# KumarRobotics/top_down_renderer

Hardware: AMD Instinct MI355X
Metric: particle-updates/sec (render+score+resample) (higher is better)
Workload: dtype f32

## Files before the change

top_down_renderer_amd/csrc/tdr_score_su.h:

```cpp
#ifndef TDR_SCORE_SU_H_
#define TDR_SCORE_SU_H_
#include "tdr_common.h"

static inline int64_t su_npad(int64_t n, int nb) { return cdiv(n + 63 * std::min<int64_t>(nb, n), 64) * 64; }
bool tdr_su_shape_ok(int nb, int nr, int group, int64_t n_total);
struct SuWs {
  int64_t tab_su, desc, bbox, keys_in, keys_out, vals_in, vals_out, ints, slots, sort_tmp, ray_tab, ray_desc, ray_multi, ray_rad, total;
  int64_t slots2, wave_tmp;
};
#define TDR_SU_TAIL_INTS 10
#define TDR_RAY_MAX_SPLIT 8
SuWs tdr_su_ws(int nb, int nr, int group, int64_t n);

struct SuLaunch {
  const tdr_map_desc* map;
  const float* tab;
  bool uniform_scale;
  const float* scan_pk;
  int nb, nr, rf;
  float res;
  const float* st;
  int64_t cap, n;
  const int32_t* perm;
  int group, nchunks;
  int64_t npad;
  float* part;
  int ray_split;
  const float* fac;
  float uscale;
  int32_t* ws;
  float span;
  float wave_span = 0.f;
};
int tdr_su_prepare(const SuLaunch& L, const SuWs& W, hipStream_t s, const int32_t** slots_out, const int32_t** counts_out);
int tdr_su_order(const SuLaunch& L, const SuWs& W, hipStream_t s, const int32_t** slots_out, const int32_t** counts_out);
struct SpanTuner {
  int64_t shape = -1;
  int phase = -2;
  int settled_launches = 0;
  int trial = 0;
  float best = 16.f;
  float round_best = 16.f, best_ms = 3.0e38f;
  hipEvent_t e0 = nullptr, e1 = nullptr;
  bool open = false, pending = false;
  int64_t trial_calls = 0;
};
float tdr_su_span_begin(SpanTuner* t, int64_t shape, hipStream_t s);
void tdr_su_span_end(SpanTuner* t, hipStream_t s);
float tdr_su_wave_span();
int tdr_su_score(const SuLaunch& L, const SuWs& W, hipStream_t s);
bool tdr_ray_map_ok(const tdr_map_desc* map);
int64_t tdr_ray_padded_samples(int nb, int nr);
int tdr_ray_splits(int nb, int nr, int64_t n, bool block_major = false);
bool tdr_ray_block_major(const SuLaunch& L);
int tdr_ray_prepare(const SuLaunch& L, const SuWs& W, hipStream_t s);
int tdr_ray_score(const SuLaunch& L, const SuWs& W, hipStream_t s);
#endif
```

top_down_renderer_amd/csrc/tdr_score_su.hip:

```cpp
#include <rocprim/device/device_radix_sort.hpp>

#include <atomic>

#include "tdr_score_dev.h"
#include "tdr_score_su.h"
#include "tdr_score_su_asm.h"

#define SU_CODE_FULL 0xFFu
#define SU_CODE_FULL_ALL 0xFEu
#define SU_CODE_PAD 0xFDu
#define SU_NSECT 8
#define SU_BOX_WORDS 4096

struct SuArgs {
  const uint32_t* crec;
  const uint32_t* kmask;
  int kcolw;
  unsigned kmask_off;
  const uint32_t* dict_int;
  int dict_n, ctiles_r;
  int pkcol;
  const int32_t* inexact;
  int rows, cols;
  float resolution;
  const float* tab_su;
  const uint32_t* desc;
  const float* bbox;
  const float* scan_pk;
  int nb, nr;
  float res;
  const float* st;
  int64_t cap;
  const int32_t* slots;
  const int32_t* nslots;
  int group, nchunks, ncls;
  int64_t npad;
  uint32_t* part;
  uint32_t* stats;
};

__global__ __launch_bounds__(256) void su_prep_kernel(const float* __restrict__ tab, const float* __restrict__ scan_pk,
                                                      int nb, int nr, int rf, int ncls, int ckconst, unsigned pbase,
                                                      unsigned plane_bytes, int group, int nchunks,
                                                      const float* __restrict__ dict, int dict_n, float* __restrict__ tab_su,
                                                      uint32_t* __restrict__ desc) {
  const int64_t t = (int64_t)blockIdx.x * blockDim.x + threadIdx.x;
  bool bad = false;
  for (int k = threadIdx.x; k < dict_n; k += blockDim.x) bad |= !(fabsf(dict[k]) <= 3.402823466e+38f);
  const bool dict_bad = __syncthreads_or(bad);
  const int64_t total = (int64_t)nchunks * nb * group;
  const bool live = t < total;
  const int64_t tt = live ? t : 0;
  const int jj = (int)(tt % group);
  const int64_t q = tt / group;
  const int i = (int)(q % nb), chunk = (int)(q / nb);
  const int j = chunk * group + jj;
  float tx = 0.f, ty = 0.f, val = 0.f;
  uint32_t code = SU_CODE_PAD, ckc = (uint32_t)ckconst, sh = 0;
  if (live && j >= nr) {
    const int64_t k = (int64_t)(nr - 1) * nb + i;
    tx = tab[2 * k];
    ty = tab[2 * k + 1];
  }
  if (live && j < nr) {
    code = 0;
    const int64_t k = (int64_t)j * nb + i;
    tx = tab[2 * k];
    ty = tab[2 * k + 1];
    const float* r = scan_pk + k * rf;
    int nz = 0, first = 0;
    bool finite = true;
    for (int c = 0; c < ncls; c++) {
      finite &= fabsf(r[c]) <= 3.402823466e+38f;
      if (r[c] != 0.f) {
        if (!nz) first = c;
        nz++;
      }
    }
    if (dict_bad || !finite) { code = SU_CODE_FULL_ALL; val = r[rf - 1]; }
    else if (nz == 1) { code = (uint32_t)first + 1u; val = r[first]; ckc = pbase + (uint32_t)first * plane_bytes; }
    else if (nz > 1) { code = SU_CODE_FULL; val = r[rf - 1]; }
  }
  uint32_t anyfull = code >= SU_CODE_FULL_ALL ? 1u : 0u;
  anyfull |= __shfl_xor(anyfull, 1);
  anyfull |= __shfl_xor(anyfull, 2);
  if (!live) return;
  tab_su[2 * t] = tx;
  tab_su[2 * t + 1] = ty;
  desc[4 * t] = code;
  desc[4 * t + 1] = (uint32_t)val;
  desc[4 * t + 2] = ckc;
  desc[4 * t + 3] = sh | (((jj & 3) == 0 && anyfull) ? 0x80000000u : 0u);
}

__global__ __launch_bounds__(256) void su_bbox_kernel(const float* __restrict__ tab_su, int nb, int nr, int group,
                                                      float* __restrict__ bbox) {
  const int chunk = blockIdx.x, sect = blockIdx.y;
  const int i0 = (int)((int64_t)sect * nb / SU_NSECT), i1 = (int)((int64_t)(sect + 1) * nb / SU_NSECT);
  const int gn = min(nr - chunk * group, group);
  float lo0 = 3.402823466e+38f, hi0 = -3.402823466e+38f, lo1 = lo0, hi1 = hi0;
  const int cnt = (i1 - i0) * gn;
  for (int t = threadIdx.x; t < cnt; t += 256) {
    const int i = i0 + t / gn, jj = t % gn;
    const float* e = tab_su + (((int64_t)chunk * nb + i) * group + jj) * 2;
    lo0 = fminf(lo0, e[0]); hi0 = fmaxf(hi0, e[0]);
    lo1 = fminf(lo1, e[1]); hi1 = fmaxf(hi1, e[1]);
  }
  __shared__ float red[4][256];
  red[0][threadIdx.x] = lo0; red[1][threadIdx.x] = hi0; red[2][threadIdx.x] = lo1; red[3][threadIdx.x] = hi1;
  __syncthreads();
  for (int d = 128; d > 0; d >>= 1) {
    if ((int)threadIdx.x < d) {
      red[0][threadIdx.x] = fminf(red[0][threadIdx.x], red[0][threadIdx.x + d]);
      red[1][threadIdx.x] = fmaxf(red[1][threadIdx.x], red[1][threadIdx.x + d]);
      red[2][threadIdx.x] = fminf(red[2][threadIdx.x], red[2][threadIdx.x + d]);
      red[3][threadIdx.x] = fmaxf(red[3][threadIdx.x], red[3][threadIdx.x + d]);
    }
    __syncthreads();
  }
  if (threadIdx.x < 4) bbox[((int64_t)chunk * SU_NSECT + sect) * 4 + threadIdx.x] = red[threadIdx.x][0];
}

__global__ __launch_bounds__(256) void su_key_kernel(const float* __restrict__ st, int64_t cap, int64_t n,
                                                     const int32_t* __restrict__ perm, int nb, float span,
                                                     uint32_t* __restrict__ keys, int32_t* __restrict__ vals,
                                                     int* __restrict__ cnt) {
  extern __shared__ int hist[];
  for (int k = threadIdx.x; k <= nb; k += 256) hist[k] = 0;
  __syncthreads();
  const int64_t t = (int64_t)blockIdx.x * blockDim.x + threadIdx.x;
  if (t < n) {
    const int32_t p = perm ? perm[t] : (int32_t)t;
    uint32_t key = (uint32_t)rot_shift_dev(st[TDR_ST_THETA * cap + p], nb);
    if (span > 0.f) {
      auto centre = [&](int64_t q, float& x, float& y) {
        const float sc = st[TDR_ST_SCALE * cap + q];
        x = st[TDR_ST_DX * cap + q] * sc + st[TDR_ST_INIT_X * cap + q];
        y = st[TDR_ST_DY * cap + q] * sc + st[TDR_ST_INIT_Y * cap + q];
      };
      const int64_t ta = t >= 32 ? t - 32 : 0, tb = t + 32 < n ? t + 32 : n - 1;
      float x0, y0, x1, y1;
      centre(perm ? perm[ta] : ta, x0, y0);
      centre(perm ? perm[tb] : tb, x1, y1);
      if (!(fabsf(x1 - x0) <= span && fabsf(y1 - y0) <= span)) key = (uint32_t)nb;
    }
    keys[t] = key;
    vals[t] = p;
    atomicAdd(&hist[key], 1);
  }
  __syncthreads();
  for (int k = threadIdx.x; k <= nb; k += 256)
    if (hist[k]) atomicAdd(&cnt[k], hist[k]);
}

__global__ __launch_bounds__(256) void su_offsets_kernel(const int* __restrict__ cnt, int nkeys, int* __restrict__ start,
                                                         int* __restrict__ slot_start, int* __restrict__ counts) {
  __shared__ int sa[256], sb[256];
  int carry_a = 0, carry_b = 0;
  for (int base = 0; base < nkeys; base += 256) {
    const int k = base + threadIdx.x;
    const int c = k < nkeys ? cnt[k] : 0;
    const int cp = k < nkeys - 1 ? (c + 63) & ~63 : c;
    sa[threadIdx.x] = c;
    sb[threadIdx.x] = cp;
    __syncthreads();
    for (int d = 1; d < 256; d <<= 1) {
      const int va = threadIdx.x >= d ? sa[threadIdx.x - d] : 0;
      const int vb = threadIdx.x >= d ? sb[threadIdx.x - d] : 0;
      __syncthreads();
      sa[threadIdx.x] += va;
      sb[threadIdx.x] += vb;
      __syncthreads();
    }
    if (k < nkeys) {
      start[k] = carry_a + sa[threadIdx.x] - c;
      slot_start[k] = carry_b + sb[threadIdx.x] - cp;
    }
    carry_a += sa[255];
    carry_b += sb[255];
    __syncthreads();
  }
  if (threadIdx.x == 0) {
    const int sparse = cnt[nkeys - 1];
    counts[0] = carry_b - sparse;
    counts[1] = sparse;
    counts[2] = carry_b;
  }
}

__global__ __launch_bounds__(256) void su_scatter_kernel(const uint32_t* __restrict__ keys, const int32_t* __restrict__ vals,
                                                         int64_t n, const int* __restrict__ start,
                                                         const int* __restrict__ slot_start, int32_t* __restrict__ slots) {
  const int64_t t = (int64_t)blockIdx.x * blockDim.x + threadIdx.x;
  if (t >= n) return;
  const uint32_t k = keys[t];
  slots[slot_start[k] + ((int)t - start[k])] = vals[t];
}

__global__ __launch_bounds__(256) void su_wave_far_kernel(const float* __restrict__ st, int64_t cap, const int32_t* __restrict__ slots,
                                                          const int32_t* __restrict__ counts, float wave_span,
                                                          int32_t* __restrict__ keep, int32_t* __restrict__ moved) {
  const int lane = threadIdx.x & 63;
  const int64_t w = (int64_t)blockIdx.x * 4 + (threadIdx.x >> 6), base = w * 64;
  if (base >= (int64_t)counts[0]) return;
  const int32_t p = slots[base + lane];
  float x0 = 3.0e38f, x1 = -3.0e38f, y0 = 3.0e38f, y1 = -3.0e38f;
  if (p >= 0) {
    const float sc = st[TDR_ST_SCALE * cap + p];
    const float x = st[TDR_ST_DX * cap + p] * sc + st[TDR_ST_INIT_X * cap + p];
    const float y = st[TDR_ST_DY * cap + p] * sc + st[TDR_ST_INIT_Y * cap + p];
    x0 = x1 = x;
    y0 = y1 = y;
  }
#pragma unroll
  for (int d = 32; d > 0; d >>= 1) {
    x0 = fminf(x0, __shfl_xor(x0, d)); x1 = fmaxf(x1, __shfl_xor(x1, d));
    y0 = fminf(y0, __shfl_xor(y0, d)); y1 = fmaxf(y1, __shfl_xor(y1, d));
  }
  const int nvalid = __popcll(__ballot(p >= 0));
  const bool far = (x1 - x0 > wave_span) || (y1 - y0 > wave_span);
  if (lane == 0) {
    keep[w] = far ? 0 : 1;
    moved[w] = far ? nvalid : 0;
  }
}
__global__ __launch_bounds__(256) void su_compact_offsets_kernel(int32_t* __restrict__ keep, int32_t* __restrict__ moved,
                                                                 int32_t* __restrict__ counts, int32_t* __restrict__ old_counts) {
  __shared__ int sa[256], sb[256];
  const int c0 = counts[0], c1 = counts[1], c2 = counts[2];
  const int nw = c0 >> 6;
  int carry_a = 0, carry_b = 0;
  for (int base = 0; base < nw; base += 256) {
    const int w = base + threadIdx.x;
    const int a = w < nw ? keep[w] : 0, b = w < nw ? moved[w] : 0;
    sa[threadIdx.x] = a;
    sb[threadIdx.x] = b;
    __syncthreads();
    for (int d = 1; d < 256; d <<= 1) {
      const int va = threadIdx.x >= d ? sa[threadIdx.x - d] : 0;
      const int vb = threadIdx.x >= d ? sb[threadIdx.x - d] : 0;
      __syncthreads();
      sa[threadIdx.x] += va;
      sb[threadIdx.x] += vb;
      __syncthreads();
    }
    if (w < nw) {
      keep[w] = a ? (carry_a + sa[threadIdx.x] - a) * 64 : -1;
      moved[w] = carry_b + sb[threadIdx.x] - b;
    }
    carry_a += sa[255];
    carry_b += sb[255];
    __syncthreads();
  }
  if (threadIdx.x == 0) {
    old_counts[0] = c0; old_counts[1] = c1; old_counts[2] = c2;
    counts[0] = carry_a * 64;
    counts[1] = c1 + carry_b;
    counts[2] = carry_a * 64 + c1 + carry_b;
  }
}
__global__ __launch_bounds__(256) void su_compact_scatter_kernel(const int32_t* __restrict__ slots, const int32_t* __restrict__ keep,
                                                                 const int32_t* __restrict__ moved,
                                                                 const int32_t* __restrict__ counts,
                                                                 const int32_t* __restrict__ old_counts, int32_t* __restrict__ out) {
  const int64_t t = (int64_t)blockIdx.x * blockDim.x + threadIdx.x;
  const int oc0 = old_counts[0], oc1 = old_counts[1];
  if (t >= (int64_t)oc0 + oc1) return;
  const int32_t p = slots[t];
  if (t >= oc0) {
    out[(int64_t)counts[0] + (t - oc0)] = p;
    return;
  }
  const int64_t w = t >> 6;
  const int32_t k = keep[w];
  const uint64_t valid = __ballot(p >= 0);
  if (k >= 0) {
    out[(int64_t)k + (t & 63)] = p;
  } else if (p >= 0) {
    const int rank = __popcll(valid & (((uint64_t)1 << (t & 63)) - 1));
    out[(int64_t)counts[0] + oc1 + moved[w] + rank] = p;
  }
}
__global__ void su_copy_slots_kernel(const int32_t* __restrict__ src, const int32_t* __restrict__ counts, int32_t* __restrict__ dst) {
  const int64_t t = (int64_t)blockIdx.x * blockDim.x + threadIdx.x;
  if (t < (int64_t)counts[2]) dst[t] = src[t];
}

struct SuLds {
  uint32_t dict[TDR_CMAP_MAX_DICT];
  uint32_t bits[SU_BOX_WORDS];
  int box[4];
};

template <int NV4, bool KSLOT, bool USCALE>
__global__ __launch_bounds__(256) __attribute__((amdgpu_waves_per_eu(6, 8))) void score_polar_su_kernel(SuArgs a) {
  constexpr int RF = 4 * NV4;
  constexpr int ND = CmapShape<RF, KSLOT>::ND, CW = CmapShape<RF, KSLOT>::CW;
  constexpr bool ASM_LOOP = CW == 2 && ND == 6;
  __shared__ SuLds lds;
  if (int_form_off(a.inexact)) return;
  for (int t = threadIdx.x; t < a.dict_n; t += 256) lds.dict[t] = a.dict_int[t];
  const int lane = threadIdx.x & 63, wave = __builtin_amdgcn_readfirstlane(threadIdx.x >> 6);
  const int64_t nsl = (int64_t)__builtin_amdgcn_readfirstlane(*a.nslots);
  if ((int64_t)blockIdx.x * 256 >= nsl) return;
  const int64_t base = ((int64_t)blockIdx.x * 4 + wave) * 64;
  const bool active = base < nsl;
  const int32_t sp = active ? a.slots[base + lane] : -1;
  const int32_t p0 = a.slots[active ? base : (int64_t)blockIdx.x * 256];
  const int64_t p = sp >= 0 ? sp : p0;
  const float scale = a.st[TDR_ST_SCALE * a.cap + p];
  const float cx = a.st[TDR_ST_DX * a.cap + p] * scale + a.st[TDR_ST_INIT_X * a.cap + p];
  const float cy = a.st[TDR_ST_DY * a.cap + p] * scale + a.st[TDR_ST_INIT_Y * a.cap + p];
  const float off0 = cy / a.resolution;
  const float off1 = cx / a.resolution;
  const int shift = __builtin_amdgcn_readfirstlane(rot_shift_dev(a.st[TDR_ST_THETA * a.cap + p], a.nb));
  const int nb = a.nb, G = a.group;
  const int j0 = blockIdx.y * G, gn = min(a.nr - j0, G);
  const float rmaxf = (float)a.rows, cmaxf = (float)a.cols;
  const int ckcol = a.ctiles_r * 128 - 16 * CW;
  const int pkcol = a.pkcol;
  const uint32_t ckconst = (uint32_t)(a.ctiles_r * 128 + 128);
  auto su_rec_const = [&](uint32_t cd) -> uint32_t {
    return cd != 0 && cd < SU_CODE_PAD ? ckconst + 4u * (((cd - 1u) * 11u) >> 5) : ckconst;
  };
  typedef const float __attribute__((address_space(4))) * tdr_const_f;
  typedef const uint32_t __attribute__((address_space(4))) * tdr_const_u;
  const tdr_const_f tbase = (tdr_const_f)a.tab_su + (int64_t)blockIdx.y * nb * G * 2;
  const tdr_const_u dbase = (tdr_const_u)a.desc + (int64_t)blockIdx.y * nb * G * 4;
  const tdr_const_f bbase = (tdr_const_f)a.bbox + (int64_t)blockIdx.y * SU_NSECT * 4;
  const tdr_const_f scanc = (tdr_const_f)a.scan_pk;
  const uint32_t* __restrict__ crec = a.crec;
  const uint32_t* __restrict__ kmask = a.kmask;
  const unsigned lds_base = (unsigned)(uintptr_t)&lds;
  const unsigned lbits_lds = (unsigned)(uintptr_t)&lds.bits[0];

  typedef float tdr_v2f __attribute__((ext_vector_type(2)));
  const tdr_v2f offv = {off0, off1};
  typedef const uint32_t __attribute__((address_space(3))) * tdr_lds_u;
  auto lds_word = [](unsigned byte_addr) -> uint32_t { return *reinterpret_cast<tdr_lds_u>((uintptr_t)byte_addr); };
  const char* __restrict__ crecb = reinterpret_cast<const char*>(a.crec);
  auto map_dword = [&](unsigned off) -> uint32_t { return *reinterpret_cast<const uint32_t*>(crecb + off); };
  auto map_ushort = [&](unsigned off) -> uint32_t { return *reinterpret_cast<const uint16_t*>(crecb + off); };
  const bool weird = !(fabsf(off0) <= 1e9f) || !(fabsf(off1) <= 1e9f) || (!USCALE && !(fabsf(scale * a.res) <= 1e9f));
  auto field = [&](const uint32_t (&w)[CW], int k) -> uint32_t {
    const uint32_t ww = w[k / 3];
    const int sh = 10 * (k % 3);
    const uint32_t boff = sh ? ((ww >> sh) & 0xFFCu) : (ww & 0xFFCu);
    return *reinterpret_cast<const uint32_t*>(reinterpret_cast<const char*>(lds.dict) + boff);
  };
  auto field1 = [&](uint32_t ww, int k) -> uint32_t {
    const int sh = 10 * (k % 3);
    const uint32_t boff = sh ? ((ww >> sh) & 0xFFCu) : (ww & 0xFFCu);
    return *reinterpret_cast<const uint32_t*>(reinterpret_cast<const char*>(lds.dict) + boff);
  };

  uint64_t acc[ND];
#pragma unroll
  for (int k = 0; k < ND; k++) acc[k] = 0;
  uint32_t norm = 0;
  uint32_t known = 0;

  auto single_class = [&](uint32_t cd, uint32_t v, uint32_t ww) {
    switch (cd) {
#define SU_CASE(K)                                                                                 \
  case K + 1:                                                                                      \
    if constexpr (K < ND) {                                                                        \
      const uint32_t m = field1(ww, K < ND ? K : 0);                                               \
      asm volatile("v_mad_u64_u32 %0, vcc, %1, %2, %0" : "+v"(acc[K < ND ? K : 0]) : "s"(v), "v"(m) : "vcc"); \
    }                                                                                              \
    break;
      SU_CASE(0) SU_CASE(1) SU_CASE(2) SU_CASE(3) SU_CASE(4) SU_CASE(5)
      SU_CASE(6) SU_CASE(7) SU_CASE(8) SU_CASE(9) SU_CASE(10)
#undef SU_CASE
      default: break;
    }
  };
  auto single_class_plane = [&](uint32_t cd, uint32_t v, uint32_t cell) {
    const uint32_t m = *reinterpret_cast<const uint32_t*>(reinterpret_cast<const char*>(lds.dict) + (cell & 0xFFCu));
    switch (cd) {
#define SU_CASE(K)                                                                                 \
  case K + 1:                                                                                      \
    if constexpr (K < ND) {                                                                        \
      asm volatile("v_mad_u64_u32 %0, vcc, %1, %2, %0" : "+v"(acc[K < ND ? K : 0]) : "s"(v), "v"(m) : "vcc"); \
    }                                                                                              \
    break;
      SU_CASE(0) SU_CASE(1) SU_CASE(2) SU_CASE(3) SU_CASE(4) SU_CASE(5)
      SU_CASE(6) SU_CASE(7) SU_CASE(8) SU_CASE(9) SU_CASE(10)
#undef SU_CASE
      default: break;
    }
  };
  auto full_bin = [&](uint32_t cd, uint32_t v, const uint32_t (&wr)[CW], int kbit, int64_t bin) {
    const tdr_const_f S = scanc + bin * RF;
    norm += v & (0u - (uint32_t)kbit);
#pragma unroll
    for (int k = 0; k < ND; k++) {
      const float sk = S[k];
      if (sk != 0.f) acc[k] += (uint64_t)(uint32_t)sk * (uint64_t)field(wr, k);
    }
  };
  auto cell = [&](float tx, float ty, int& ri, int& ci) {
    tdr_v2f pv = {tx, ty};
    if constexpr (!USCALE) pv = (pv * scale) * a.res;
    pv = pv + offv;
    tdr_v2f qv = {__builtin_amdgcn_fmed3f(pv.x, -1.f, rmaxf), __builtin_amdgcn_fmed3f(pv.y, -1.f, cmaxf)};
    qv = qv + 0.49999997f;
    asm("v_cvt_flr_i32_f32 %0, %1" : "=v"(ri) : "v"(qv.x));
    asm("v_cvt_flr_i32_f32 %0, %1" : "=v"(ci) : "v"(qv.y));
  };

  auto cpp_step = [&](int i, int r, int jj, int krow4, int kconst) {
    const tdr_const_f T = tbase + ((int64_t)i * G + jj) * 2;
    const tdr_const_u D = dbase + ((int64_t)r * G + jj) * 4;
    uint32_t val[4];
    uint32_t code[4], pad[4];
    uint32_t w[4], bits[4];
    int cis[4];
    unsigned offs[4];
#pragma unroll
    for (int u = 0; u < 4; u++) {
      code[u] = D[4 * u];
      pad[u] = code[u] == SU_CODE_PAD ? 0u : 0xFFFFFFFFu;
      code[u] = code[u] == SU_CODE_PAD ? 0u : code[u];
      val[u] = D[4 * u + 1];
      const uint32_t ckc = su_rec_const(code[u]);
      int ri, ci;
      cell(T[2 * u], T[2 * u + 1], ri, ci);
      cis[u] = ci;
      int wa;
      asm("v_mad_i32_i24 %0, %1, %2, %3" : "=v"(wa) : "v"(ri), "v"(krow4), "s"(kconst));
      const int cw5 = ci >> 5;
      unsigned la;
      asm("v_lshl_add_u32 %0, %1, 2, %2" : "=v"(la) : "v"(cw5), "v"(wa));
      bits[u] = lds_word(la);
      w[u] = 0;
      offs[u] = 0;
      if (code[u] != 0) {
        int t1, t2;
        const int cq = ci >> 2;
        asm("v_mad_i32_i24 %0, %1, %2, %3" : "=v"(t1) : "v"(cq), "v"(ckcol), "s"(ckc));
        asm("v_lshl_add_u32 %0, %1, %2, %3" : "=v"(t2) : "v"(ci), "n"(CW == 1 ? 2 : (CW == 2 ? 3 : 4)), "v"(t1));
        asm("v_lshl_add_u32 %0, %1, %2, %3" : "=v"(offs[u]) : "v"(ri), "n"(CW == 1 ? 4 : (CW == 2 ? 5 : 6)), "v"(t2));
        w[u] = map_dword(offs[u]);
      }
    }
#pragma unroll
    for (int u = 0; u < 4; u++) {
      const uint32_t cd = code[u];
      int kmsk;
      asm("v_bfe_i32 %0, %1, %2, 1" : "=v"(kmsk) : "v"(bits[u]), "v"(cis[u]));
      known -= (uint32_t)kmsk & pad[u];
      if (cd != 0) {
        if (cd < SU_CODE_FULL_ALL) {
          norm += (uint32_t)kmsk & val[u];
          single_class(cd, val[u], w[u]);
        } else {
          uint32_t wr[CW];
          wr[0] = w[u];
#pragma unroll
          for (int d = 1; d < CW; d++)
            wr[d] = map_dword(offs[u] + 4u * d);
          full_bin(cd, val[u], wr, kmsk & 1, (int64_t)(j0 + jj + u) * nb + r);
        }
      }
    }
  };
  auto cpp_step_plane = [&](int i, int r, int jj, int krow4, int kconst) {
    const tdr_const_f T = tbase + ((int64_t)i * G + jj) * 2;
    const tdr_const_u D = dbase + ((int64_t)r * G + jj) * 4;
    uint32_t val[4];
    uint32_t code[4], pad[4];
    uint32_t w[4], bits[4];
    int cis[4];
#pragma unroll
    for (int u = 0; u < 4; u++) {
      code[u] = D[4 * u];
      pad[u] = code[u] == SU_CODE_PAD ? 0u : 0xFFFFFFFFu;
      code[u] = code[u] == SU_CODE_PAD ? 0u : code[u];
      val[u] = D[4 * u + 1];
      const uint32_t pkc = D[4 * u + 2];
      int ri, ci;
      cell(T[2 * u], T[2 * u + 1], ri, ci);
      cis[u] = ci;
      int wa;
      asm("v_mad_i32_i24 %0, %1, %2, %3" : "=v"(wa) : "v"(ri), "v"(krow4), "s"(kconst));
      const int cw5 = ci >> 5;
      unsigned la;
      asm("v_lshl_add_u32 %0, %1, 2, %2" : "=v"(la) : "v"(cw5), "v"(wa));
      bits[u] = lds_word(la);
      w[u] = 0;
      if (code[u] != 0) {
        int t1, t2;
        unsigned off;
        const int cq = ci >> 3;
        asm("v_mad_i32_i24 %0, %1, %2, %3" : "=v"(t1) : "v"(cq), "v"(pkcol), "s"(pkc));
        asm("v_lshl_add_u32 %0, %1, 1, %2" : "=v"(t2) : "v"(ci), "v"(t1));
        asm("v_lshl_add_u32 %0, %1, 4, %2" : "=v"(off) : "v"(ri), "v"(t2));
        w[u] = map_ushort(off);
      }
// ... 36 lines not shown
          const uint32_t ckc = su_rec_const(D[4 * u]);
          int t1, t2;
          const int cq = ci >> 2;
          asm("v_mad_i32_i24 %0, %1, %2, %3" : "=v"(t1) : "v"(cq), "v"(ckcol), "s"(ckc));
          asm("v_lshl_add_u32 %0, %1, %2, %3" : "=v"(t2) : "v"(ci), "n"(CW == 1 ? 2 : (CW == 2 ? 3 : 4)), "v"(t1));
          asm("v_lshl_add_u32 %0, %1, %2, %3" : "=v"(off) : "v"(ri), "n"(CW == 1 ? 4 : (CW == 2 ? 5 : 6)), "v"(t2));
        }
        w[4 * d + u] = map_dword(off);
      }
      jx += 4;
      if (jx >= ((gn + 3) & ~3)) { jx = 0; ii++; }
    }
    ii = i; jx = jj;
#pragma unroll
    for (int d = 0; d < NS; d++) {
      int r = ii + shift;
      r -= r >= nb ? nb : 0;
      const tdr_const_u D = dbase + ((int64_t)r * G + jx) * 4;
#pragma unroll
      for (int u = 0; u < 4; u++) {
        const uint32_t ww = w[4 * d + u];
        const uint32_t cdr = D[4 * u];
        const uint32_t cd = cdr == SU_CODE_PAD ? 0u : cdr;
        const int sidx = 4 * d + u;
        const uint32_t kb = cd == 0 ? (ww >> ((cbits[sidx / 6] >> (5 * (sidx % 6))) & 31u)) & 1u : (ww & 1u);
        known += cdr == SU_CODE_PAD ? 0u : kb;
        if (cd != 0) {
          const uint32_t v = D[4 * u + 1];
          if (cd < SU_CODE_FULL_ALL) {
            norm += (0u - kb) & v;
            single_class(cd, v, ww);
          } else {
            int iq = ii;
            asm volatile("" : "+s"(iq));
            const tdr_const_f T = tbase + ((int64_t)iq * G + jx) * 2;
            int ri, ci;
            cell(T[2 * u], T[2 * u + 1], ri, ci);
            const unsigned off = cmap_offset<CW, (CW == 1 ? 3 : (CW == 2 ? 2 : 1))>(ri, ci, ckcol, a.ctiles_r * 128 + 128);
            uint32_t wr[CW];
            wr[0] = ww;
#pragma unroll
            for (int q = 1; q < CW; q++)
              wr[q] = map_dword(off + 4u * q);
            full_bin(cd, v, wr, (int)kb, (int64_t)(j0 + jx + u) * nb + r);
          }
        }
      }
      jx += 4;
      if (jx >= ((gn + 3) & ~3)) { jx = 0; ii++; }
    }
  };
  constexpr int FAR_DEPTH = 4;
  auto far_sector = [&](int i0, int i1) {
    const int gn4 = (gn + 3) & ~3;
    const int spd = gn4 >> 2, total = (i1 - i0) * spd;
    int i = i0, jj = 0, k = 0;
    auto advance = [&](int steps) {
      jj += 4 * steps;
      while (jj >= gn4) { jj -= gn4; i++; }
    };
    for (; k + FAR_DEPTH <= total; k += FAR_DEPTH) {
      far_steps(std::integral_constant<int, FAR_DEPTH>{}, i, jj);
      advance(FAR_DEPTH);
    }
    for (; k < total; k++) {
      far_steps(std::integral_constant<int, 1>{}, i, jj);
      advance(1);
    }
  };
  auto run_sector = [&](int i0, int i1, int krow4, int kconst, bool inside, bool allknown) {
    if constexpr (ASM_LOOP) {
      if (gn == G && lds_base == 0 && (G == 4 || G == 8 || G == 16)) {
        const int spd = G / 4;
        int r0 = i0 + shift;
        r0 -= r0 >= nb ? nb : 0;
        uint32_t toff = __builtin_amdgcn_readfirstlane((uint32_t)i0 * (uint32_t)G * 8u);
        uint32_t doff = __builtin_amdgcn_readfirstlane((uint32_t)r0 * (uint32_t)G * 16u);
        uint32_t nleft = __builtin_amdgcn_readfirstlane((uint32_t)((i1 - i0) * spd - 1));
        uint32_t wleft = __builtin_amdgcn_readfirstlane((uint32_t)((nb - r0) * spd - 1));
        const uint32_t wrapm1 = __builtin_amdgcn_readfirstlane((uint32_t)(nb * spd - 1));
        const int kconst_s = __builtin_amdgcn_readfirstlane(kconst);
        const uint64_t half2 = 0x3EFFFFFF3EFFFFFFull;
        const float rmax_s = __uint_as_float(__builtin_amdgcn_readfirstlane(__float_as_uint(rmaxf)));
        const float cmax_s = __uint_as_float(__builtin_amdgcn_readfirstlane(__float_as_uint(cmaxf)));
        const tdr_v2f scale2 = {scale, scale};
        const uint64_t res2 = (uint64_t)__float_as_uint(a.res) * 0x100000001ull;
        while (nleft != 0xFFFFFFFFu) {
#define SU_ASM_OPERANDS                                                                                               \
                          \
          : [a0] "+{v[32:33]}"(acc[0]), [a1] "+{v[34:35]}"(acc[1]), [a2] "+{v[36:37]}"(acc[2]), [a3] "+{v[38:39]}"(acc[3]),    \
            [a4] "+{v[40:41]}"(acc[4]), [a5] "+{v[42:43]}"(acc[ND > 5 ? 5 : 0]), [norm] "+v"(norm), [known] "+v"(known),       \
            [toff] "+v"(toff), [doff] "+v"(doff),                                                                             \
            [nleft] "+v"(nleft), [wleft] "+v"(wleft)                                                                   \
          : [offv] "v"(offv), [krow4] "v"(krow4), [pkcol] "v"(pkcol), [tb] "s"(tbase), [db] "s"(dbase),              \
            [rmax] "s"(rmax_s), [cmax] "s"(cmax_s), [half] "s"(half2), [kconst] "s"(kconst_s), [crec] "s"(crec),           \
            [wrapm1] "s"(wrapm1), [scale2] "v"(scale2), [res2] "s"(res2)                                               \
          : SU_ASM_CLOBBERS
          if (allknown) {
            if constexpr (USCALE) asm volatile(SU_ASM_US_ALLKNOWN SU_ASM_OPERANDS);
            else asm volatile(SU_ASM_PS_ALLKNOWN SU_ASM_OPERANDS);
          } else if (inside) {
            if constexpr (USCALE) asm volatile(SU_ASM_US_NOCLAMP SU_ASM_OPERANDS);
            else asm volatile(SU_ASM_PS_NOCLAMP SU_ASM_OPERANDS);
          } else {
            if constexpr (USCALE) asm volatile(SU_ASM_US SU_ASM_OPERANDS);
            else asm volatile(SU_ASM_PS SU_ASM_OPERANDS);
          }
#undef SU_ASM_OPERANDS
          toff = __builtin_amdgcn_readfirstlane(toff); doff = __builtin_amdgcn_readfirstlane(doff);
          nleft = __builtin_amdgcn_readfirstlane(nleft); wleft = __builtin_amdgcn_readfirstlane(wleft);
          if (nleft == 0xFFFFFFFFu) break;
          const int k = (i1 - i0) * spd - 1 - (int)nleft, lsp = G == 4 ? 0 : (G == 8 ? 1 : 2);
          const int i = i0 + (k >> lsp), jj = (k & (spd - 1)) * 4;
          int r = i + shift;
          r -= r >= nb ? nb : 0;
          cpp_step(i, r, jj, krow4, kconst);
          toff += 32u;
          doff += 64u;
          if (wleft == 0) { doff = 0; wleft = wrapm1; } else wleft--;
          nleft--;
          toff = __builtin_amdgcn_readfirstlane(toff); doff = __builtin_amdgcn_readfirstlane(doff);
          nleft = __builtin_amdgcn_readfirstlane(nleft); wleft = __builtin_amdgcn_readfirstlane(wleft);
        }
        return;
      }
    }
    for (int i = i0; i < i1; i++) {
      int r = i + shift;
      r -= r >= nb ? nb : 0;
      for (int jj = 0; jj < gn; jj += 4) {
        if (dbase[((int64_t)r * G + jj) * 4 + 3] >> 31) cpp_step(i, r, jj, krow4, kconst);
        else cpp_step_plane(i, r, jj, krow4, kconst);
      }
    }
  };

  for (int sect = 0; sect < SU_NSECT; sect++) {
    const int i0 = (int)((int64_t)sect * nb / SU_NSECT), i1 = (int)((int64_t)(sect + 1) * nb / SU_NSECT);
    float a0 = bbase[4 * sect], b0 = bbase[4 * sect + 1], a1 = bbase[4 * sect + 2], b1 = bbase[4 * sect + 3];
    if constexpr (!USCALE) {
      const float x0 = (a0 * scale) * a.res, y0 = (b0 * scale) * a.res, x1 = (a1 * scale) * a.res, y1 = (b1 * scale) * a.res;
      a0 = fminf(x0, y0); b0 = fmaxf(x0, y0); a1 = fminf(x1, y1); b1 = fmaxf(x1, y1);
    }
    int rl = (int)fminf(fmaxf(floorf(a0 + off0) - 1.f, -1.f), rmaxf), rh = (int)fminf(fmaxf(ceilf(b0 + off0) + 1.f, -1.f), rmaxf);
    int cl = (int)fminf(fmaxf(floorf(a1 + off1) - 1.f, -1.f), cmaxf), ch = (int)fminf(fmaxf(ceilf(b1 + off1) + 1.f, -1.f), cmaxf);
    if (weird) { rl = -1; rh = a.rows; cl = -1; ch = a.cols; }
    if (!active) { rl = 0x7FFFFFFF; rh = -0x7FFFFFFF; cl = 0x7FFFFFFF; ch = -0x7FFFFFFF; }
#pragma unroll
    for (int d = 32; d > 0; d >>= 1) {
      rl = min(rl, __shfl_xor(rl, d)); rh = max(rh, __shfl_xor(rh, d));
      cl = min(cl, __shfl_xor(cl, d)); ch = max(ch, __shfl_xor(ch, d));
    }
    __syncthreads();
    if (threadIdx.x == 0) { lds.box[0] = 0x7FFFFFFF; lds.box[1] = -0x7FFFFFFF; lds.box[2] = 0x7FFFFFFF; lds.box[3] = -0x7FFFFFFF; }
    __syncthreads();
    if (lane == 0 && active) {
      atomicMin(&lds.box[0], rl); atomicMax(&lds.box[1], rh); atomicMin(&lds.box[2], cl); atomicMax(&lds.box[3], ch);
    }
    __syncthreads();
    const int rlo = __builtin_amdgcn_readfirstlane(lds.box[0]), rhi = __builtin_amdgcn_readfirstlane(lds.box[1]);
    const int wlo = (__builtin_amdgcn_readfirstlane(lds.box[2]) >> 5) + 1;
    const int whi = (__builtin_amdgcn_readfirstlane(lds.box[3]) >> 5) + 1;
    const int H = rhi - rlo + 1, Wb = whi - wlo + 1;
    const bool fits = (int64_t)H * Wb <= SU_BOX_WORDS;
    uint32_t every = 0xFFFFFFFFu;
    if (fits) {
      const int total = H * Wb;
      for (int idx = threadIdx.x; idx < total; idx += 256) {
        const int wc = idx / H, row = idx - wc * H;
        const uint32_t wv = kmask[(int64_t)(wlo + wc) * a.kcolw + (rlo + row + 32)];
        lds.bits[row * Wb + wc] = wv;
        every &= wv;
      }
    }
    const bool allknown = __syncthreads_and(fits && every == 0xFFFFFFFFu);
    if (active) {
      const bool inside = rlo >= 0 && rhi < a.rows && __builtin_amdgcn_readfirstlane(lds.box[2]) >= 0 &&
                          __builtin_amdgcn_readfirstlane(lds.box[3]) < a.cols;
      int box_krow4 = Wb * 4, box_kconst = (int)lbits_lds + (1 - wlo - rlo * Wb) * 4;
      int box_ok = fits ? 1 : 0, box_inside = inside ? 1 : 0, box_allknown = allknown ? 1 : 0;
      if (!fits) {
        const int wrl = __builtin_amdgcn_readfirstlane(rl), wrh = __builtin_amdgcn_readfirstlane(rh);
        const int wcl = __builtin_amdgcn_readfirstlane(cl), wch = __builtin_amdgcn_readfirstlane(ch);
        const int wl = (wcl >> 5) + 1, wh = (wch >> 5) + 1;
        const int Hw = wrh - wrl + 1, Wbw = wh - wl + 1;
        if ((int64_t)Hw * Wbw <= SU_BOX_WORDS / 4) {
          uint32_t* const mine = lds.bits + wave * (SU_BOX_WORDS / 4);
          uint32_t ev = 0xFFFFFFFFu;
          const int total = Hw * Wbw;
          for (int idx = lane; idx < total; idx += 64) {
            const int wc = idx / Hw, row = idx - wc * Hw;
            const uint32_t wv = kmask[(int64_t)(wl + wc) * a.kcolw + (wrl + row + 32)];
            mine[row * Wbw + wc] = wv;
            ev &= wv;
          }
          __builtin_amdgcn_fence(__ATOMIC_RELEASE, "wavefront");
          __builtin_amdgcn_wave_barrier();
          box_ok = 1;
          box_krow4 = Wbw * 4;
          box_kconst = (int)lbits_lds + wave * (SU_BOX_WORDS / 4) * 4 + (1 - wl - wrl * Wbw) * 4;
          box_inside = (wrl >= 0 && wrh < a.rows && wcl >= 0 && wch < a.cols) ? 1 : 0;
          box_allknown = __all(ev == 0xFFFFFFFFu) ? 1 : 0;
        }
      }
      box_ok = __builtin_amdgcn_readfirstlane(box_ok);
      box_inside = __builtin_amdgcn_readfirstlane(box_inside);
      box_allknown = __builtin_amdgcn_readfirstlane(box_allknown);
      box_krow4 = __builtin_amdgcn_readfirstlane(box_krow4);
      box_kconst = __builtin_amdgcn_readfirstlane(box_kconst);
      if (a.stats && lane == 0)
        atomicAdd(&a.stats[!box_ok ? 6 : ((fits ? 0 : 3) + (box_allknown ? 0 : (box_inside ? 1 : 2)))], 1u);
      if (box_ok) run_sector(i0, i1, box_krow4, box_kconst, box_inside != 0, box_allknown != 0);
      else far_sector(i0, i1);
    }
  }
  if (active) {
    const int64_t slot = base + lane;
    uint32_t* o = a.part + (int64_t)blockIdx.y * (2 * a.ncls + 2) * a.npad + slot;
#pragma unroll
    for (int k = 0; k < ND; k++)
      if (k < a.ncls) {
        o[(int64_t)(2 * k) * a.npad] = (uint32_t)acc[k];
        o[(int64_t)(2 * k + 1) * a.npad] = (uint32_t)(acc[k] >> 32);
      }
    o[(int64_t)(2 * a.ncls) * a.npad] = norm;
    o[(int64_t)(2 * a.ncls + 1) * a.npad] = known;
  }
}

static int g_su_mode = 1;
extern "C" int tdr_config_shift_uniform(int mode) {
  if (mode >= 0) g_su_mode = mode > 2 ? 2 : mode;
  return g_su_mode;
}
extern "C" size_t tdr_cmap_tile_words(int ncls, int rows, int cols);
extern "C" size_t tdr_cmap_plane_offset_words(int ncls, int rows, int cols);
extern "C" size_t tdr_cmap_plane_words(int ncls, int rows, int cols);
#define SU_SPAN_START 16.f
static bool g_su_span_fixed = false;
static float g_su_span = SU_SPAN_START;
extern "C" float tdr_config_shift_uniform_span(float cells) {
  if (cells >= 0.f) { g_su_span = cells; g_su_span_fixed = true; }
  else if (cells < -1.5f) { g_su_span = SU_SPAN_START; g_su_span_fixed = false; }
  return g_su_span;
}
namespace {
constexpr float kSpanCand[] = {2.f, 8.f, 16.f, 24.f, 40.f};
constexpr int kSpanCands = (int)(sizeof(kSpanCand) / sizeof(kSpanCand[0]));
constexpr int kSpanTrials = 2;
constexpr int kSpanSkip = 30;
constexpr int kSpanRetune = 4000;
}
float tdr_su_span_begin(SpanTuner* t, int64_t shape, hipStream_t s) {
  if (g_su_span_fixed || !t) return g_su_span;
  if (!t->e0 && (hipEventCreate(&t->e0) != hipSuccess || hipEventCreate(&t->e1) != hipSuccess)) return g_su_span;
  if (shape != t->shape) { t->shape = shape; t->phase = -kSpanSkip; t->trial = 0; t->best_ms = 3.0e38f; t->pending = false; t->best = t->round_best = g_su_span; }
  if (t->pending) {
    if (hipEventQuery(t->e1) != hipSuccess) return t->best;
    float ms = 0.f;
    if (hipEventElapsedTime(&ms, t->e0, t->e1) == hipSuccess && ms > 0.f && ms < t->best_ms) {
      t->best_ms = ms;
      t->round_best = kSpanCand[t->phase];
    }
    t->pending = false;
    if (++t->trial >= kSpanTrials) { t->trial = 0; t->phase++; }
    if (t->phase >= kSpanCands) { t->settled_launches = 0; t->best = t->round_best; }
  }
  if (t->phase < 0) { t->phase++; return t->best; }
  if (t->phase >= kSpanCands) {
    if (++t->settled_launches < kSpanRetune) return t->best;
    t->phase = 0;
    t->best_ms = 3.0e38f;
    t->round_best = t->best;
  }
  t->open = hipEventRecord(t->e0, s) == hipSuccess;
  t->trial_calls++;
  return kSpanCand[t->phase];
}
void tdr_su_span_end(SpanTuner* t, hipStream_t s) {
  if (g_su_span_fixed || !t || !t->open) return;
  t->open = false;
  t->pending = hipEventRecord(t->e1, s) == hipSuccess;
}
static float g_su_wave_span = 0.f;
extern "C" int tdr_config_su_wave_span(int cells) {
  if (cells >= 0) g_su_wave_span = (float)cells;
  return (int)g_su_wave_span;
}
float tdr_su_wave_span() { return g_su_wave_span; }
static int g_su_lds_pad = 0;
extern "C" int tdr_config_su_lds_pad(int bytes) {
  if (bytes >= 0) g_su_lds_pad = bytes;
  return g_su_lds_pad;
}
static std::atomic<int64_t> g_su_launches{0};
extern "C" int64_t tdr_shift_uniform_launches(void) { return g_su_launches.load(); }
bool tdr_su_shape_ok(int nb, int nr, int group, int64_t n_total) {
  if (g_su_mode == 0) return false;
  if (group % 4 != 0 || nb > 4095) return false;
  if (g_su_mode == 2) return true;
  if ((int64_t)nb * nr < 8192) return false;
  return n_total >= (int64_t)64 * nb;
}
static size_t su_sort_tmp_bytes(int64_t n) {
  size_t bytes = 0;
  uint32_t* k = nullptr;
  int32_t* v = nullptr;
  hipError_t e = rocprim::radix_sort_pairs(nullptr, bytes, k, k, v, v, (size_t)std::max<int64_t>(n, 1), 0u, 12u,
                                           (hipStream_t)0, false);
  if (e != hipSuccess || bytes == 0) bytes = (size_t)(n + 4096) * 16;
  return bytes;
}
SuWs tdr_su_ws(int nb, int nr, int group, int64_t n) {
  SuWs w;
  const int64_t nchunks = cdiv(nr, group), nbins = nchunks * nb * group;
  int64_t o = 0;
  auto take = [&](int64_t words) { const int64_t at = o; o += (words + 63) / 64 * 64; return at; };
  w.tab_su = take(2 * nbins);
  w.desc = take(4 * nbins);
  w.bbox = take(nchunks * SU_NSECT * 4);
  w.keys_in = take(n);
  w.keys_out = take(n);
  w.vals_in = take(n);
  w.vals_out = take(n);
  w.ints = take(3 * ((int64_t)nb + 1) + TDR_SU_TAIL_INTS);
  w.slots = take(su_npad(n, nb));
  w.slots2 = take(su_npad(n, nb));
  w.wave_tmp = take(2 * (su_npad(n, nb) / 64 + 1));
  w.sort_tmp = take((int64_t)((su_sort_tmp_bytes(n) + 3) / 4));
  const int64_t T = tdr_ray_padded_samples(nb, nr);
  w.ray_tab = take(2 * T);
  w.ray_desc = take((T + 1) / 2);
  w.ray_multi = take((int64_t)nb * nr);
  w.ray_rad = take(T / nb);
  w.total = o;
  return w;
}

int tdr_su_order(const SuLaunch& L, const SuWs& W, hipStream_t s, const int32_t** slots_out, const int32_t** counts_out) {
  int32_t* base = L.ws;
  uint32_t* keys_in = reinterpret_cast<uint32_t*>(base + W.keys_in);
  uint32_t* keys_out = reinterpret_cast<uint32_t*>(base + W.keys_out);
  int32_t* vals_in = base + W.vals_in;
  int32_t* vals_out = base + W.vals_out;
  int* cnt = base + W.ints;
  const int nkeys = L.nb + 1;
  int* start = cnt + nkeys;
  int* slot_start = start + nkeys;
  int* counts = slot_start + nkeys;
  int32_t* slots = base + W.slots;
  const int64_t n = L.n;
  HIP_TRY(hipMemsetAsync(cnt, 0, sizeof(int) * (size_t)(3 * nkeys + TDR_SU_TAIL_INTS), s));
  HIP_TRY(hipMemsetAsync(slots, 0xFF, sizeof(int32_t) * (size_t)L.npad, s));
  hipLaunchKernelGGL(su_key_kernel, dim3((unsigned)cdiv(n, 256)), dim3(256), sizeof(int) * (size_t)nkeys, s, L.st, L.cap, n,
                     L.perm, L.nb, L.span, keys_in, vals_in, cnt);
  LAUNCH_CHECK("su_key");
  hipLaunchKernelGGL(su_offsets_kernel, dim3(1), dim3(256), 0, s, (const int*)cnt, nkeys, start, slot_start, counts);
  LAUNCH_CHECK("su_offsets");
  unsigned bits = 1;
  while ((1u << bits) < (unsigned)nkeys) bits++;
  size_t tmp_bytes = su_sort_tmp_bytes(n);
  HIP_TRY(rocprim::radix_sort_pairs(base + W.sort_tmp, tmp_bytes, keys_in, keys_out, vals_in, vals_out, (size_t)n, 0u, bits,
                                    s, false));
  hipLaunchKernelGGL(su_scatter_kernel, dim3((unsigned)cdiv(n, 256)), dim3(256), 0, s, (const uint32_t*)keys_out,
                     (const int32_t*)vals_out, n, (const int*)start, (const int*)slot_start, slots);
  LAUNCH_CHECK("su_scatter");
  if (L.wave_span > 0.f && L.nb > 1) {
    int32_t* slots2 = base + W.slots2;
    int32_t* keep = base + W.wave_tmp;
    int32_t* moved = keep + (L.npad / 64 + 1);
    int32_t* old_counts = counts + 7;
    const int64_t nwaves = L.npad / 64;
    hipLaunchKernelGGL(su_wave_far_kernel, dim3((unsigned)cdiv(nwaves, 4)), dim3(256), 0, s, L.st, L.cap, (const int32_t*)slots,
                       (const int32_t*)counts, L.wave_span, keep, moved);
    hipLaunchKernelGGL(su_compact_offsets_kernel, dim3(1), dim3(256), 0, s, keep, moved, counts, old_counts);
    hipLaunchKernelGGL(su_compact_scatter_kernel, dim3((unsigned)cdiv(L.npad, 256)), dim3(256), 0, s, (const int32_t*)slots,
                       (const int32_t*)keep, (const int32_t*)moved, (const int32_t*)counts, (const int32_t*)old_counts, slots2);
    hipLaunchKernelGGL(su_copy_slots_kernel, dim3((unsigned)cdiv(L.npad, 256)), dim3(256), 0, s, (const int32_t*)slots2,
                       (const int32_t*)counts, slots);
    LAUNCH_CHECK("su_reroute");
  }
  *slots_out = slots;
  *counts_out = counts;
  return TDR_OK;
}
int tdr_su_prepare(const SuLaunch& L, const SuWs& W, hipStream_t s, const int32_t** slots_out, const int32_t** counts_out) {
  if (int rc = tdr_su_order(L, W, s, slots_out, counts_out)) return rc;
  int32_t* base = L.ws;
  float* tab_su = reinterpret_cast<float*>(base + W.tab_su);
  uint32_t* desc = reinterpret_cast<uint32_t*>(base + W.desc);
  const int64_t ndesc = (int64_t)L.nchunks * L.nb * L.group;
  const int lc = L.map->cwords == 1 ? 3 : (L.map->cwords == 2 ? 2 : 1);
  const int ckconst = ((L.map->rows >> lc) + 2) * 128 + 128;
  const unsigned plane_bytes = (unsigned)(tdr_cmap_plane_words(L.map->ncls, L.map->rows, L.map->cols) * 4);
  const unsigned pbase = (unsigned)(tdr_cmap_plane_offset_words(L.map->ncls, L.map->rows, L.map->cols) * 4) +
                         (unsigned)(plane_trows(L.map->rows) * 128) + 128u;
  hipLaunchKernelGGL(su_prep_kernel, dim3((unsigned)cdiv(ndesc, 256)), dim3(256), 0, s, L.tab, L.scan_pk, L.nb, L.nr, L.rf,
                     L.map->ncls, ckconst, pbase, plane_bytes, L.group, L.nchunks, L.map->dict, L.map->dict_n, tab_su, desc);
  LAUNCH_CHECK("su_prep");
  hipLaunchKernelGGL(su_bbox_kernel, dim3((unsigned)L.nchunks, SU_NSECT), dim3(256), 0, s, (const float*)tab_su, L.nb, L.nr,
                     L.group, reinterpret_cast<float*>(base + W.bbox));
  LAUNCH_CHECK("su_bbox");
  return TDR_OK;
}

int tdr_su_score(const SuLaunch& L, const SuWs& W, hipStream_t s) {
  const tdr_map_desc* map = L.map;
  int32_t* base = L.ws;
  int* nslots = base + W.ints + 3 * (L.nb + 1);
  SuArgs u;
  const int lc = map->cwords == 1 ? 3 : (map->cwords == 2 ? 2 : 1);
  u.crec = map->crec; u.dict_int = reinterpret_cast<const uint32_t*>(map->dict) + TDR_CMAP_MAX_DICT;
  u.dict_n = map->dict_n; u.ctiles_r = (map->rows >> lc) + 2;
  u.pkcol = plane_trows(map->rows) * 128 - 16;
  u.inexact = nslots + 4;
  u.rows = map->rows; u.cols = map->cols; u.resolution = map->resolution;
  u.tab_su = reinterpret_cast<const float*>(base + W.tab_su);
  u.desc = reinterpret_cast<const uint32_t*>(base + W.desc);
  u.bbox = reinterpret_cast<const float*>(base + W.bbox);
  u.kmask = map->crec + tdr_cmap_tile_words(map->ncls, map->rows, map->cols);
  u.kcolw = kmask_trows(map->rows) * 32;
  u.kmask_off = (unsigned)(tdr_cmap_tile_words(map->ncls, map->rows, map->cols) * 4);
  u.scan_pk = L.scan_pk;
  u.nb = L.nb; u.nr = L.nr; u.res = L.res; u.st = L.st; u.cap = L.cap;
  u.slots = base + W.slots; u.nslots = nslots;
  u.group = L.group; u.nchunks = L.nchunks; u.ncls = map->ncls; u.npad = L.npad; u.part = reinterpret_cast<uint32_t*>(L.part);
  u.stats = tdr_profile_stats_ptr();
  const dim3 grid((unsigned)cdiv(L.npad, 256), (unsigned)L.nchunks), block(256);
  const bool ks = tdr_has_kslot(map->ncls, L.rf), us = L.uniform_scale;
#define TDR_LAUNCH_SU(NV4)                                                                         \
  if (ks && us) hipLaunchKernelGGL((score_polar_su_kernel<NV4, true, true>), grid, block, g_su_lds_pad, s, u);  \
  else if (ks) hipLaunchKernelGGL((score_polar_su_kernel<NV4, true, false>), grid, block, g_su_lds_pad, s, u);  \
  else if (us) hipLaunchKernelGGL((score_polar_su_kernel<NV4, false, true>), grid, block, g_su_lds_pad, s, u);  \
  else hipLaunchKernelGGL((score_polar_su_kernel<NV4, false, false>), grid, block, g_su_lds_pad, s, u);
  switch (L.rf / 4) {
    case 1: TDR_LAUNCH_SU(1) break;
    case 2: TDR_LAUNCH_SU(2) break;
    case 3: TDR_LAUNCH_SU(3) break;
    default: return fail(TDR_ERR_ARG, "score: no shift-uniform kernel for record size %d", L.rf);
  }
#undef TDR_LAUNCH_SU
  LAUNCH_CHECK("score_polar_su");
  g_su_launches.fetch_add(1);
  return TDR_OK;
}
```

Before: 22.48 million.

## Replace rocprim radix sort with fused tile-count ranking scatter for particle ordering

Removes the rocprim radix_sort_pairs call, the separate offsets kernel and both memsets. Instead, the key kernel writes per-tile histograms, and one scatter kernel does several jobs: it computes each tile's prefix across tiles and a global exclusive scan, ranks keys within the tile using wave ballots (a stable counting sort), writes the slots directly, and fills the padding with -1. This cuts launches and the multi-pass sort traffic. In exchange, every scatter block redundantly scans all tile counts, which costs O(ntiles*nkeys) work per block.

```diff
diff --git a/top_down_renderer_amd/csrc/tdr_score_su.h b/top_down_renderer_amd/csrc/tdr_score_su.h
--- a/top_down_renderer_amd/csrc/tdr_score_su.h
+++ b/top_down_renderer_amd/csrc/tdr_score_su.h
@@ -5,7 +5,7 @@
 static inline int64_t su_npad(int64_t n, int nb) { return cdiv(n + 63 * std::min<int64_t>(nb, n), 64) * 64; }
 bool tdr_su_shape_ok(int nb, int nr, int group, int64_t n_total);
 struct SuWs {
-  int64_t tab_su, desc, bbox, keys_in, keys_out, vals_in, vals_out, ints, slots, sort_tmp, ray_tab, ray_desc, ray_multi, ray_rad, total;
+  int64_t tab_su, desc, bbox, keys, tile_cnt, ints, slots, ray_tab, ray_desc, ray_multi, ray_rad, total;
   int64_t slots2, wave_tmp;
 };
 #define TDR_SU_TAIL_INTS 10
diff --git a/top_down_renderer_amd/csrc/tdr_score_su.hip b/top_down_renderer_amd/csrc/tdr_score_su.hip
--- a/top_down_renderer_amd/csrc/tdr_score_su.hip
+++ b/top_down_renderer_amd/csrc/tdr_score_su.hip
@@ -1,10 +1,9 @@
-#include <rocprim/device/device_radix_sort.hpp>
-
 #include <atomic>
 
 #include "tdr_score_dev.h"
 #include "tdr_score_su.h"
 #include "tdr_score_su_asm.h"
+#include "tdr_tile_rank.h"
 
 #define SU_CODE_FULL 0xFFu
 #define SU_CODE_FULL_ALL 0xFEu
@@ -121,12 +120,16 @@
   if (threadIdx.x < 4) bbox[((int64_t)chunk * SU_NSECT + sect) * 4 + threadIdx.x] = red[threadIdx.x][0];
 }
 
+#define SU_TILE_IPT 8
+#define SU_TILE (256 * SU_TILE_IPT)
 __global__ __launch_bounds__(256) void su_key_kernel(const float* __restrict__ st, int64_t cap, int64_t n,
                                                      const int32_t* __restrict__ perm, int nb, float span,
-                                                     uint32_t* __restrict__ keys, int32_t* __restrict__ vals,
-                                                     int* __restrict__ cnt) {
+                                                     uint32_t* __restrict__ keys, int* __restrict__ tile_cnt,
+                                                     int* __restrict__ tail) {
   extern __shared__ int hist[];
-  for (int k = threadIdx.x; k <= nb; k += 256) hist[k] = 0;
+  const int nkeys = nb + 1;
+  for (int k = threadIdx.x; k < nkeys; k += 256) hist[k] = 0;
+  if (blockIdx.x == 0 && threadIdx.x < TDR_SU_TAIL_INTS) tail[threadIdx.x] = 0;
   __syncthreads();
   const int64_t t = (int64_t)blockIdx.x * blockDim.x + threadIdx.x;
   if (t < n) {
@@ -145,21 +148,38 @@
       if (!(fabsf(x1 - x0) <= span && fabsf(y1 - y0) <= span)) key = (uint32_t)nb;
     }
     keys[t] = key;
-    vals[t] = p;
     atomicAdd(&hist[key], 1);
   }
   __syncthreads();
-  for (int k = threadIdx.x; k <= nb; k += 256)
-    if (hist[k]) atomicAdd(&cnt[k], hist[k]);
-}
-
-__global__ __launch_bounds__(256) void su_offsets_kernel(const int* __restrict__ cnt, int nkeys, int* __restrict__ start,
-                                                         int* __restrict__ slot_start, int* __restrict__ counts) {
+  int* row = tile_cnt + (int64_t)(blockIdx.x / SU_TILE_IPT) * nkeys;
+  for (int k = threadIdx.x; k < nkeys; k += 256)
+    if (hist[k]) atomicAdd(&row[k], hist[k]);
+}
+
+__global__ __launch_bounds__(256) void su_scatter_kernel(const uint32_t* __restrict__ keys, const int32_t* __restrict__ perm,
+                                                         int64_t n, int nb, const int* __restrict__ tile_cnt, int ntiles,
+                                                         int64_t npad, int* __restrict__ cnt, int* __restrict__ start,
+                                                         int* __restrict__ slot_start, int* __restrict__ counts,
+                                                         int32_t* __restrict__ slots) {
+  extern __shared__ int lds[];
+  const int nkeys = nb + 1;
+  int* run = lds;
+  int* pre = run + 4 * nkeys;
+  int* tot = pre + nkeys;
+  int* sst = tot + nkeys;
   __shared__ int sa[256], sb[256];
+  for (int k = threadIdx.x; k < 4 * nkeys; k += 256) run[k] = 0;
+  for (int k = threadIdx.x; k < nkeys; k += 256) {
+    int a = 0, c = 0;
+    tile_sums(tile_cnt + k, nkeys, ntiles, a, c);
+    pre[k] = a;
+    tot[k] = c;
+  }
+  __syncthreads();
   int carry_a = 0, carry_b = 0;
   for (int base = 0; base < nkeys; base += 256) {
     const int k = base + threadIdx.x;
-    const int c = k < nkeys ? cnt[k] : 0;
+    const int c = k < nkeys ? tot[k] : 0;
     const int cp = k < nkeys - 1 ? (c + 63) & ~63 : c;
     sa[threadIdx.x] = c;
     sb[threadIdx.x] = cp;
@@ -173,28 +193,51 @@
       __syncthreads();
     }
     if (k < nkeys) {
-      start[k] = carry_a + sa[threadIdx.x] - c;
-      slot_start[k] = carry_b + sb[threadIdx.x] - cp;
+      sst[k] = carry_b + sb[threadIdx.x] - cp;
+      if (blockIdx.x == 0) {
+        cnt[k] = c;
+        start[k] = carry_a + sa[threadIdx.x] - c;
+        slot_start[k] = sst[k];
+      }
     }
     carry_a += sa[255];
     carry_b += sb[255];
     __syncthreads();
   }
-  if (threadIdx.x == 0) {
-    const int sparse = cnt[nkeys - 1];
+  if (blockIdx.x == 0 && threadIdx.x == 0) {
+    const int sparse = tot[nkeys - 1];
     counts[0] = carry_b - sparse;
     counts[1] = sparse;
     counts[2] = carry_b;
   }
-}
-
-__global__ __launch_bounds__(256) void su_scatter_kernel(const uint32_t* __restrict__ keys, const int32_t* __restrict__ vals,
-                                                         int64_t n, const int* __restrict__ start,
-                                                         const int* __restrict__ slot_start, int32_t* __restrict__ slots) {
-  const int64_t t = (int64_t)blockIdx.x * blockDim.x + threadIdx.x;
-  if (t >= n) return;
-  const uint32_t k = keys[t];
-  slots[slot_start[k] + ((int)t - start[k])] = vals[t];
+  for (int k = threadIdx.x; k < nkeys - 1; k += 256)
+    if (k % ntiles == (int)blockIdx.x)
+      for (int j = sst[k] + tot[k], e = sst[k] + ((tot[k] + 63) & ~63); j < e; j++) slots[j] = -1;
+  for (int64_t j = (int64_t)carry_b + (int64_t)blockIdx.x * 256 + threadIdx.x; j < npad; j += (int64_t)ntiles * 256) slots[j] = -1;
+  int nbits = 1;
+  while ((1 << nbits) < nkeys) nbits++;
+  const int64_t t0 = (int64_t)blockIdx.x * SU_TILE + (threadIdx.x >> 6) * (64 * SU_TILE_IPT) + (threadIdx.x & 63);
+  uint32_t key[SU_TILE_IPT];
+  bool valid[SU_TILE_IPT];
+  int rank[SU_TILE_IPT];
+#pragma unroll
+  for (int r = 0; r < SU_TILE_IPT; r++) {
+    const int64_t t = t0 + r * 64;
+    valid[r] = t < n;
+    key[r] = valid[r] ? keys[t] : 0u;
+  }
+  tile_rank<SU_TILE_IPT>(key, valid, nbits, run, nkeys, rank);
+  __syncthreads();
+  tile_wave_offsets(run, nkeys);
+  __syncthreads();
+  const int* wrun = run + (threadIdx.x >> 6) * nkeys;
+#pragma unroll
+  for (int r = 0; r < SU_TILE_IPT; r++) {
+    if (!valid[r]) continue;
+    const int64_t t = t0 + r * 64;
+    const uint32_t k = key[r];
+    slots[(int64_t)sst[k] + pre[k] + wrun[k] + rank[r]] = perm ? perm[t] : (int32_t)t;
+  }
 }
 
 __global__ __launch_bounds__(256) void su_wave_far_kernel(const float* __restrict__ st, int64_t cap, const int32_t* __restrict__ slots,
@@ -837,15 +880,6 @@
   if ((int64_t)nb * nr < 8192) return false;
   return n_total >= (int64_t)64 * nb;
 }
-static size_t su_sort_tmp_bytes(int64_t n) {
-  size_t bytes = 0;
-  uint32_t* k = nullptr;
-  int32_t* v = nullptr;
-  hipError_t e = rocprim::radix_sort_pairs(nullptr, bytes, k, k, v, v, (size_t)std::max<int64_t>(n, 1), 0u, 12u,
-                                           (hipStream_t)0, false);
-  if (e != hipSuccess || bytes == 0) bytes = (size_t)(n + 4096) * 16;
-  return bytes;
-}
 SuWs tdr_su_ws(int nb, int nr, int group, int64_t n) {
   SuWs w;
   const int64_t nchunks = cdiv(nr, group), nbins = nchunks * nb * group;
@@ -854,15 +888,12 @@
   w.tab_su = take(2 * nbins);
   w.desc = take(4 * nbins);
   w.bbox = take(nchunks * SU_NSECT * 4);
-  w.keys_in = take(n);
-  w.keys_out = take(n);
-  w.vals_in = take(n);
-  w.vals_out = take(n);
+  w.keys = take(n);
+  w.tile_cnt = take(cdiv(std::max<int64_t>(n, 1), SU_TILE) * ((int64_t)nb + 1));
   w.ints = take(3 * ((int64_t)nb + 1) + TDR_SU_TAIL_INTS);
   w.slots = take(su_npad(n, nb));
   w.slots2 = take(su_npad(n, nb));
   w.wave_tmp = take(2 * (su_npad(n, nb) / 64 + 1));
-  w.sort_tmp = take((int64_t)((su_sort_tmp_bytes(n) + 3) / 4));
   const int64_t T = tdr_ray_padded_samples(nb, nr);
   w.ray_tab = take(2 * T);
   w.ray_desc = take((T + 1) / 2);
@@ -874,10 +905,8 @@
 
 int tdr_su_order(const SuLaunch& L, const SuWs& W, hipStream_t s, const int32_t** slots_out, const int32_t** counts_out) {
   int32_t* base = L.ws;
-  uint32_t* keys_in = reinterpret_cast<uint32_t*>(base + W.keys_in);
-  uint32_t* keys_out = reinterpret_cast<uint32_t*>(base + W.keys_out);
-  int32_t* vals_in = base + W.vals_in;
-  int32_t* vals_out = base + W.vals_out;
+  uint32_t* keys = reinterpret_cast<uint32_t*>(base + W.keys);
+  int* tile_cnt = base + W.tile_cnt;
   int* cnt = base + W.ints;
   const int nkeys = L.nb + 1;
   int* start = cnt + nkeys;
@@ -885,20 +914,14 @@
   int* counts = slot_start + nkeys;
   int32_t* slots = base + W.slots;
   const int64_t n = L.n;
-  HIP_TRY(hipMemsetAsync(cnt, 0, sizeof(int) * (size_t)(3 * nkeys + TDR_SU_TAIL_INTS), s));
-  HIP_TRY(hipMemsetAsync(slots, 0xFF, sizeof(int32_t) * (size_t)L.npad, s));
-  hipLaunchKernelGGL(su_key_kernel, dim3((unsigned)cdiv(n, 256)), dim3(256), sizeof(int) * (size_t)nkeys, s, L.st, L.cap, n,
-                     L.perm, L.nb, L.span, keys_in, vals_in, cnt);
+  const int ntiles = (int)std::max<int64_t>(cdiv(n, SU_TILE), 1);
+  HIP_TRY(hipMemsetAsync(tile_cnt, 0, sizeof(int) * (size_t)ntiles * (size_t)nkeys, s));
+  hipLaunchKernelGGL(su_key_kernel, dim3((unsigned)std::max<int64_t>(cdiv(n, 256), 1)), dim3(256), sizeof(int) * (size_t)nkeys,
+                     s, L.st, L.cap, n, L.perm, L.nb, L.span, keys, tile_cnt, counts);
   LAUNCH_CHECK("su_key");
-  hipLaunchKernelGGL(su_offsets_kernel, dim3(1), dim3(256), 0, s, (const int*)cnt, nkeys, start, slot_start, counts);
-  LAUNCH_CHECK("su_offsets");
-  unsigned bits = 1;
-  while ((1u << bits) < (unsigned)nkeys) bits++;
-  size_t tmp_bytes = su_sort_tmp_bytes(n);
-  HIP_TRY(rocprim::radix_sort_pairs(base + W.sort_tmp, tmp_bytes, keys_in, keys_out, vals_in, vals_out, (size_t)n, 0u, bits,
-                                    s, false));
-  hipLaunchKernelGGL(su_scatter_kernel, dim3((unsigned)cdiv(n, 256)), dim3(256), 0, s, (const uint32_t*)keys_out,
-                     (const int32_t*)vals_out, n, (const int*)start, (const int*)slot_start, slots);
+  hipLaunchKernelGGL(su_scatter_kernel, dim3((unsigned)ntiles), dim3(256), sizeof(int) * 7 * (size_t)nkeys, s,
+                     (const uint32_t*)keys, L.perm, n, L.nb, (const int*)tile_cnt, ntiles, L.npad, cnt, start, slot_start,
+                     counts, slots);
   LAUNCH_CHECK("su_scatter");
   if (L.wave_span > 0.f && L.nb > 1) {
     int32_t* slots2 = base + W.slots2;
diff --git a/top_down_renderer_amd/csrc/tdr_tile_rank.h b/top_down_renderer_amd/csrc/tdr_tile_rank.h
--- /dev/null
+++ b/top_down_renderer_amd/csrc/tdr_tile_rank.h
@@ -0,0 +1,57 @@
+#pragma once
+#include <hip/hip_runtime.h>
+#include <stdint.h>
+
+__device__ __forceinline__ uint64_t tile_peers(uint32_t d, bool valid, int nbits) {
+  uint64_t m = __ballot(valid);
+  for (int b = 0; b < nbits; b++) {
+    const bool bit = (d >> b) & 1u;
+    const uint64_t x = __ballot(bit);
+    m &= bit ? x : ~x;
+  }
+  return valid ? m : 0ull;
+}
+
+template <int IPT>
+__device__ __forceinline__ void tile_rank(const uint32_t (&dig)[IPT], const bool (&valid)[IPT], int nbits, int* run,
+                                          int nbins, int (&rank)[IPT]) {
+  const int lane = threadIdx.x & 63;
+  int* wrun = run + (threadIdx.x >> 6) * nbins;
+  const uint64_t below_mask = (1ull << lane) - 1ull;
+#pragma unroll
+  for (int r = 0; r < IPT; r++) {
+    const uint64_t m = tile_peers(dig[r], valid[r], nbits);
+    const int below = __popcll(m & below_mask);
+    int old = 0;
+    if (valid[r] && below == 0) {
+      old = wrun[dig[r]];
+      wrun[dig[r]] = old + __popcll(m);
+    }
+    const int leader = m ? __ffsll((unsigned long long)m) - 1 : lane;
+    old = __shfl(old, leader);
+    rank[r] = old + below;
+  }
+}
+
+__device__ __forceinline__ void tile_wave_offsets(int* run, int nbins) {
+  for (int d = threadIdx.x; d < nbins; d += blockDim.x) {
+    const int c0 = run[d], c1 = run[nbins + d], c2 = run[2 * nbins + d];
+    run[d] = 0;
+    run[nbins + d] = c0;
+    run[2 * nbins + d] = c0 + c1;
+    run[3 * nbins + d] = c0 + c1 + c2;
+  }
+}
+
+__device__ __forceinline__ void tile_sums(const int* __restrict__ col, int stride, int ntiles, int& before, int& total) {
+  for (int b0 = 0; b0 < ntiles; b0 += 16) {
+    int v[16];
+#pragma unroll
+    for (int j = 0; j < 16; j++) v[j] = b0 + j < ntiles ? col[(int64_t)(b0 + j) * stride] : 0;
+#pragma unroll
+    for (int j = 0; j < 16; j++) {
+      before += b0 + j < (int)blockIdx.x ? v[j] : 0;
+      total += v[j];
+    }
+  }
+}
```

Result: faster. 22.81 million (median of 6 runs) (+1.5%).
